# yflyzhang/RankPO

Hardware: AMD Instinct MI355X
Metric: query-passage pairs/sec (higher is better)
Workload: dtype bf16

## Files before the change

rankpo_amd/csrc/encoder_ops.hip:

```cpp
#include "common.hpp"

namespace {

constexpr int kEwThreads = 256;

__device__ __forceinline__ float sigmoid_f(float x) { return 1.0f / (1.0f + __expf(-x)); }

template <typename T>
__global__ __launch_bounds__(kEwThreads) void swiglu_fwd_kernel(const T* __restrict__ g, const T* __restrict__ u,
                                                                T* __restrict__ out, int64_t rows, int vec_per_row,
                                                                int64_t ld_gu, int64_t ld_out) {
    constexpr int V = Elem<T>::kVec;
    const int64_t i = (int64_t)blockIdx.x * kEwThreads + threadIdx.x;
    const int64_t r = i / vec_per_row;
    if (r >= rows) return;
    const int c = (int)(i - r * vec_per_row) * V;
    Vec16<T> a, b, o;
    a.load_nt(g + r * ld_gu + c);
    b.load_nt(u + r * ld_gu + c);
#pragma unroll
    for (int k = 0; k < V; ++k) o.v[k] = a.v[k] * sigmoid_f(a.v[k]) * b.v[k];
    o.store_nt(out + r * ld_out + c);
}

template <typename T>
__global__ __launch_bounds__(kEwThreads) void swiglu_bwd_kernel(const T* g, const T* u, const T* dout, T* dg, T* du,
                                                                T* prod, int64_t rows, int vec_per_row, int64_t ld_gu,
                                                                int64_t ld_dout, int64_t ld_dgu,
                                                                int64_t ld_prod) {
    constexpr int V = Elem<T>::kVec;
    const int64_t i = (int64_t)blockIdx.x * kEwThreads + threadIdx.x;
    const int64_t r = i / vec_per_row;
    if (r >= rows) return;
    const int c = (int)(i - r * vec_per_row) * V;
    Vec16<T> a, b, d, og, ou, op;
    a.load_nt(g + r * ld_gu + c);
    b.load_nt(u + r * ld_gu + c);
    d.load_nt(dout + r * ld_dout + c);
#pragma unroll
    for (int k = 0; k < V; ++k) {
        const float s = sigmoid_f(a.v[k]);
        const float silu = a.v[k] * s;
        og.v[k] = d.v[k] * b.v[k] * (s + silu * (1.0f - s));
        ou.v[k] = d.v[k] * silu;
        op.v[k] = silu * b.v[k];
    }
    og.store_nt(dg + r * ld_dgu + c);
    ou.store_nt(du + r * ld_dgu + c);
    if (prod) op.store_nt(prod + r * ld_prod + c);
}

template <typename T>
__global__ __launch_bounds__(kEwThreads) void rope_kernel(const T* xin, T* x, int64_t row_stride,
                                                          const float* __restrict__ cs, const float* __restrict__ sn,
                                                          int64_t rows, int H, int hd, int64_t period, float sign) {
    constexpr int V = Elem<T>::kVec;
    const int half = hd >> 1;
    const int vec_per_head = half / V;
    const int total = H * vec_per_head;
    const int rpb = total <= kEwThreads / 2 ? kEwThreads / total : 1;
    const int rin = rpb > 1 ? threadIdx.x / total : 0;
    const int i0 = rpb > 1 ? threadIdx.x - rin * total : threadIdx.x;
    if (rin >= rpb) return;
    for (int64_t r = (int64_t)blockIdx.x * rpb + rin; r < rows; r += (int64_t)gridDim.x * rpb) {
        T* xr = x + r * row_stride;
        const T* xi = xin + r * row_stride;
        const float* c = cs + (r % period) * half;
        const float* s = sn + (r % period) * half;
        for (int i = i0; i < total; i += (rpb > 1 ? total : kEwThreads)) {
            const int h = i / vec_per_head, j = (i - h * vec_per_head) * V;
            T* lo = xr + h * hd + j;
            T* hi = lo + half;
            Vec16<T> a, b, oa, ob;
            a.load_nt(xi + h * hd + j);
            b.load_nt(xi + h * hd + j + half);
#pragma unroll
            for (int k = 0; k < V; ++k) {
                const float cc = c[j + k], ss = sign * s[j + k];
                oa.v[k] = a.v[k] * cc - b.v[k] * ss;
                ob.v[k] = b.v[k] * cc + a.v[k] * ss;
            }
            oa.store_nt(lo);
            ob.store_nt(hi);
        }
    }
}

template <typename T, int TC, bool DGU_T>
__global__ __launch_bounds__(256) void swiglu_bwd_t_kernel(const T* __restrict__ g, const T* __restrict__ u, const T* __restrict__ dout,
                                                           T* __restrict__ dg, T* __restrict__ du, T* __restrict__ prod_t,
                                                           T* __restrict__ dgu_t, int64_t rows, int64_t cols, int64_t ld_gu,
                                                           int64_t ld_dout, int64_t ld_dgu, int64_t ld_pt) {
    constexpr int V = Elem<T>::kVec;
    constexpr int TR = 64;
    constexpr int LDT = TC + 8 / (int)sizeof(T);
    constexpr int VPR = TC / V;
    constexpr int VPC = TR / V;
    constexpr int NI = TR * VPR / 256;
    __shared__ __attribute__((aligned(16))) T tile[TR][LDT];
    const int64_t r0 = (int64_t)blockIdx.y * TR, c0 = (int64_t)blockIdx.x * TC;
    const int t = threadIdx.x;
    auto st_tile = [](T* dst, const uint4_t v) {
        uint2_t* d2 = reinterpret_cast<uint2_t*>(dst);
        d2[0] = uint2_t{v.x, v.y};
        d2[1] = uint2_t{v.z, v.w};
    };
    uint4_t pk_g[DGU_T ? NI : 1], pk_u[DGU_T ? NI : 1];
#pragma unroll
    for (int i = 0; i < NI; ++i) {
        const int idx = t + 256 * i;
        const int row = idx / VPR, cv = (idx % VPR) * V;
        const int64_t r = r0 + row, c = c0 + cv;
        __attribute__((aligned(16))) T pv[V];
        __attribute__((aligned(16))) T gv[V];
        __attribute__((aligned(16))) T uv[V];
        if (r < rows && c < cols) {
            Vec16<T> a, b, d, og, ou;
            a.load_nt(g + r * ld_gu + c);
            b.load_nt(u + r * ld_gu + c);
            d.load_nt(dout + r * ld_dout + c);
#pragma unroll
            for (int k = 0; k < V; ++k) {
                const float sg = sigmoid_f(a.v[k]);
                const float silu = a.v[k] * sg;
                og.v[k] = d.v[k] * b.v[k] * (sg + silu * (1.0f - sg));
                ou.v[k] = d.v[k] * silu;
                Elem<T>::st(&pv[k], silu * b.v[k]);
                if constexpr (DGU_T) {
                    Elem<T>::st(&gv[k], og.v[k]);
                    Elem<T>::st(&uv[k], ou.v[k]);
                }
            }
            og.store_nt(dg + r * ld_dgu + c);
            ou.store_nt(du + r * ld_dgu + c);
        } else {
#pragma unroll
            for (int k = 0; k < V; ++k) pv[k] = gv[k] = uv[k] = T(0);
        }
        st_tile(&tile[row][cv], *reinterpret_cast<const uint4_t*>(pv));
        if constexpr (DGU_T) {
            pk_g[i] = *reinterpret_cast<const uint4_t*>(gv);
            pk_u[i] = *reinterpret_cast<const uint4_t*>(uv);
        }
    }
    auto flush = [&](T* __restrict__ out) {
        __syncthreads();
#pragma unroll
        for (int i = 0; i < TC * VPC / 256; ++i) {
            const int idx = t + 256 * i;
            const int oc = idx / VPC, rv = (idx % VPC) * V;
            const int64_t c = c0 + oc, r = r0 + rv;
            if (c >= cols || r >= rows) continue;
            __attribute__((aligned(16))) T v[V];
#pragma unroll
            for (int e = 0; e < V; ++e) v[e] = tile[rv + e][oc];
            if (r + V <= rows) {
                __builtin_nontemporal_store(*reinterpret_cast<const uint4_t*>(v), reinterpret_cast<uint4_t*>(out + c * ld_pt + r));
            } else {
#pragma unroll
                for (int e = 0; e < V; ++e)
                    if (r + e < rows) out[c * ld_pt + r + e] = v[e];
            }
        }
    };
    flush(prod_t);
    if constexpr (DGU_T) {
        auto refill = [&](const uint4_t* pk) {
            __syncthreads();
#pragma unroll
            for (int i = 0; i < NI; ++i) {
                const int idx = t + 256 * i;
                st_tile(&tile[idx / VPR][(idx % VPR) * V], pk[i]);
            }
        };
        refill(pk_g);
        flush(dgu_t);
        refill(pk_u);
        flush(dgu_t + cols * ld_pt);
    }
}

inline unsigned ew_grid(int64_t nvec) { return (unsigned)rpo_cdiv(nvec, kEwThreads); }

}

template <typename T>
__global__ __launch_bounds__(256) void transpose_kernel(const T* __restrict__ in, T* __restrict__ out, int64_t R, int64_t C,
                                                        int64_t ld_in, int64_t ld_out, int vec_in, int vec_out) {
    constexpr int V = 16 / (int)sizeof(T);
    constexpr int TS = 64;
    constexpr int LDT = TS + 8 / (int)sizeof(T);
    constexpr int VPR = TS / V;
    __shared__ __attribute__((aligned(16))) T tile[TS][LDT];
    const int64_t r0 = (int64_t)blockIdx.y * TS, c0 = (int64_t)blockIdx.x * TS;
    const int t = threadIdx.x;
#pragma unroll
    for (int i = 0; i < TS * VPR / 256; ++i) {
        const int idx = t + 256 * i;
        const int row = idx / VPR, cv = (idx % VPR) * V;
        const int64_t r = r0 + row, c = c0 + cv;
        __attribute__((aligned(16))) T v[V];
        if (r < R && vec_in && c + V <= C) {
            *reinterpret_cast<uint4_t*>(v) = __builtin_nontemporal_load(reinterpret_cast<const uint4_t*>(in + r * ld_in + c));
        } else {
#pragma unroll
            for (int e = 0; e < V; ++e) v[e] = (r < R && c + e < C) ? in[r * ld_in + c + e] : T(0);
        }
#pragma unroll
        for (int e = 0; e < V; ++e) tile[row][cv + e] = v[e];
    }
    __syncthreads();
#pragma unroll
    for (int i = 0; i < TS * VPR / 256; ++i) {
        const int idx = t + 256 * i;
        const int oc = idx / VPR, rv = (idx % VPR) * V;
        const int64_t c = c0 + oc, r = r0 + rv;
        if (c >= C) continue;
        __attribute__((aligned(16))) T v[V];
#pragma unroll
        for (int e = 0; e < V; ++e) v[e] = tile[rv + e][oc];
        if (vec_out && r + V <= R) {
            __builtin_nontemporal_store(*reinterpret_cast<const uint4_t*>(v), reinterpret_cast<uint4_t*>(out + c * ld_out + r));
        } else {
#pragma unroll
            for (int e = 0; e < V; ++e)
                if (r + e < R) out[c * ld_out + r + e] = v[e];
        }
    }
}

extern "C" int rpo_transpose(const void* in, void* out, int64_t rows, int64_t cols, int64_t ld_in, int64_t ld_out, int dtype,
                             rpo_stream_t stream) {
    if (!in || !out || rows <= 0 || cols <= 0 || ld_in < cols || ld_out < rows) return RPO_ERR_INVALID_ARG;
    if (!rpo_dtype_ok(dtype)) return RPO_ERR_INVALID_ARG;
    if (dtype == RPO_DT_F16) dtype = RPO_DT_BF16;
    const int64_t gx = rpo_cdiv(cols, 64), gy = rpo_cdiv(rows, 64);
    if (gy > 65535) return RPO_ERR_UNSUPPORTED;
    const int es = dtype == RPO_DT_BF16 ? 2 : 4, V = 16 / es;
    const int vec_in = rpo_aligned16(in) && (ld_in % V == 0), vec_out = rpo_aligned16(out) && (ld_out % V == 0);
    hipStream_t st = (hipStream_t)stream;
    const dim3 grid((unsigned)gx, (unsigned)gy);
    if (dtype == RPO_DT_BF16)
        RPO_LAUNCH(transpose_kernel<bf16_t>, grid, dim3(256), 0, st, (const bf16_t*)in, (bf16_t*)out, rows, cols, ld_in, ld_out,
                   vec_in, vec_out);
    else
        RPO_LAUNCH(transpose_kernel<float>, grid, dim3(256), 0, st, (const float*)in, (float*)out, rows, cols, ld_in, ld_out,
                   vec_in, vec_out);
    return rpo_launch_status();
}

extern "C" int rpo_swiglu_fwd(const void* g, const void* u, void* out, int64_t rows, int64_t cols, int64_t ld_gu,
                              int64_t ld_out, int dtype, rpo_stream_t stream) {
    if (!g || !u || !out || rows <= 0 || cols <= 0) return RPO_ERR_INVALID_ARG;
    const int V = dtype == RPO_DT_BF16 ? 8 : 4;
    if (cols % V != 0 || ld_gu % V != 0 || ld_out % V != 0 || ld_gu < cols || ld_out < cols || !rpo_aligned16(g) ||
        !rpo_aligned16(u) || !rpo_aligned16(out))
        return RPO_ERR_UNSUPPORTED;
    const int64_t nvec = rows * (cols / V);
    if (nvec / kEwThreads >= INT32_MAX) return RPO_ERR_UNSUPPORTED;
    hipStream_t st = (hipStream_t)stream;
    if (dtype == RPO_DT_BF16)
        RPO_LAUNCH(swiglu_fwd_kernel<bf16_t>, dim3(ew_grid(nvec)), dim3(kEwThreads), 0, st, (const bf16_t*)g,
                   (const bf16_t*)u, (bf16_t*)out, rows, (int)(cols / V), ld_gu, ld_out);
    else if (dtype == RPO_DT_F32)
        RPO_LAUNCH(swiglu_fwd_kernel<float>, dim3(ew_grid(nvec)), dim3(kEwThreads), 0, st, (const float*)g,
                   (const float*)u, (float*)out, rows, (int)(cols / V), ld_gu, ld_out);
    else
        return RPO_ERR_INVALID_ARG;
    return rpo_launch_status();
}

extern "C" int rpo_swiglu_bwd(const void* g, const void* u, const void* dout, void* dg, void* du, void* prod_out,
                              int64_t rows, int64_t cols, int64_t ld_gu, int64_t ld_dout, int64_t ld_dgu, int64_t ld_prod,
                              int dtype, rpo_stream_t stream) {
    if (!g || !u || !dout || !dg || !du || rows <= 0 || cols <= 0) return RPO_ERR_INVALID_ARG;
    const int V = dtype == RPO_DT_BF16 ? 8 : 4;
    if (cols % V != 0 || ld_gu % V != 0 || ld_dout % V != 0 || ld_dgu % V != 0 || !rpo_aligned16(g) ||
        !rpo_aligned16(u) || !rpo_aligned16(dout) || !rpo_aligned16(dg) || !rpo_aligned16(du) ||
        (prod_out && (ld_prod % V != 0 || !rpo_aligned16(prod_out))))
        return RPO_ERR_UNSUPPORTED;
    const int64_t nvec = rows * (cols / V);
    if (nvec / kEwThreads >= INT32_MAX) return RPO_ERR_UNSUPPORTED;
    hipStream_t st = (hipStream_t)stream;
    if (dtype == RPO_DT_BF16)
        RPO_LAUNCH(swiglu_bwd_kernel<bf16_t>, dim3(ew_grid(nvec)), dim3(kEwThreads), 0, st, (const bf16_t*)g,
                   (const bf16_t*)u, (const bf16_t*)dout, (bf16_t*)dg, (bf16_t*)du, (bf16_t*)prod_out, rows, (int)(cols / V),
                   ld_gu, ld_dout, ld_dgu, ld_prod);
    else if (dtype == RPO_DT_F32)
        RPO_LAUNCH(swiglu_bwd_kernel<float>, dim3(ew_grid(nvec)), dim3(kEwThreads), 0, st, (const float*)g,
                   (const float*)u, (const float*)dout, (float*)dg, (float*)du, (float*)prod_out, rows, (int)(cols / V), ld_gu,
                   ld_dout, ld_dgu, ld_prod);
    else
        return RPO_ERR_INVALID_ARG;
    return rpo_launch_status();
}

extern "C" int rpo_swiglu_bwd_t(const void* g, const void* u, const void* dout, void* dg, void* du, void* prod_t_out,
                                void* dgu_t_out, int64_t rows, int64_t cols, int64_t ld_gu, int64_t ld_dout, int64_t ld_dgu,
                                int64_t ld_t, int dtype, rpo_stream_t stream) {
    if (!g || !u || !dout || !dg || !du || !prod_t_out || rows <= 0 || cols <= 0) return RPO_ERR_INVALID_ARG;
    const int V = dtype == RPO_DT_BF16 ? 8 : 4;
    if (cols % V != 0 || ld_gu % V != 0 || ld_dout % V != 0 || ld_dgu % V != 0 || ld_t % V != 0 || ld_t < rows ||
        !rpo_aligned16(g) || !rpo_aligned16(u) || !rpo_aligned16(dout) || !rpo_aligned16(dg) || !rpo_aligned16(du) ||
        !rpo_aligned16(prod_t_out) || (dgu_t_out && !rpo_aligned16(dgu_t_out)))
        return RPO_ERR_UNSUPPORTED;
    constexpr int kTC = 256;
    const int64_t gy = rpo_cdiv(rows, 64);
    if (gy > 65535) return RPO_ERR_UNSUPPORTED;
    hipStream_t st = (hipStream_t)stream;
#define RPO_SWT(T, TCV, FLAG)                                                                                               \
    RPO_LAUNCH((swiglu_bwd_t_kernel<T, TCV, FLAG>), dim3((unsigned)rpo_cdiv(cols, TCV), (unsigned)gy), dim3(256), 0, st,    \
               (const T*)g, (const T*)u, (const T*)dout, (T*)dg, (T*)du, (T*)prod_t_out, (T*)dgu_t_out, rows, cols, ld_gu,   \
               ld_dout, ld_dgu, ld_t)
    if (dtype == RPO_DT_BF16) {
        if (dgu_t_out) RPO_SWT(bf16_t, kTC, true);
        else RPO_SWT(bf16_t, kTC, false);
    } else if (dtype == RPO_DT_F32) {
        if (dgu_t_out) RPO_SWT(float, kTC / 2, true);
        else RPO_SWT(float, kTC / 2, false);
    } else {
        return RPO_ERR_INVALID_ARG;
    }
#undef RPO_SWT
    return rpo_launch_status();
}

extern "C" int rpo_rope(const void* x_in, void* x, int64_t row_stride, const float* cos_tab, const float* sin_tab, int64_t rows,
                                int64_t heads, int64_t head_dim, int64_t period, int dtype, int backward,
                                rpo_stream_t stream) {
    if (!x_in || !x || !cos_tab || !sin_tab || rows <= 0 || heads <= 0 || head_dim <= 0 || period <= 0)
        return RPO_ERR_INVALID_ARG;
    const int V = dtype == RPO_DT_BF16 ? 8 : 4;
    if ((head_dim / 2) % V != 0 || head_dim % 2 != 0 || row_stride % V != 0 || !rpo_aligned16(x) || !rpo_aligned16(x_in))
        return RPO_ERR_UNSUPPORTED;
    const int64_t pairs = heads * ((head_dim / 2) / V);
    const int64_t rpb = pairs <= kEwThreads / 2 ? kEwThreads / pairs : 1;
    const int64_t nblk = rpo_cdiv(rows, rpb);
    int64_t grid = nblk < INT32_MAX ? nblk : INT32_MAX;
    hipStream_t st = (hipStream_t)stream;
    const float sign = backward ? -1.0f : 1.0f;
    if (dtype == RPO_DT_BF16)
        RPO_LAUNCH(rope_kernel<bf16_t>, dim3((unsigned)grid), dim3(kEwThreads), 0, st, (const bf16_t*)x_in, (bf16_t*)x, row_stride, cos_tab,
                   sin_tab, rows, (int)heads, (int)head_dim, period, sign);
    else if (dtype == RPO_DT_F32)
        RPO_LAUNCH(rope_kernel<float>, dim3((unsigned)grid), dim3(kEwThreads), 0, st, (const float*)x_in, (float*)x, row_stride, cos_tab,
                   sin_tab, rows, (int)heads, (int)head_dim, period, sign);
    else
        return RPO_ERR_INVALID_ARG;
    return rpo_launch_status();
}

namespace {

constexpr int kNormThreads = 256, kNormWaves = kNormThreads / 64;

template <typename T> struct Raw16 {
    uint4_t r;
    __device__ __forceinline__ void load_nt(const T* p) { r = __builtin_nontemporal_load(reinterpret_cast<const uint4_t*>(p)); }
    __device__ __forceinline__ void load(const T* p) { r = *reinterpret_cast<const uint4_t*>(p); }
    __device__ __forceinline__ float get(int e) const;
};
template <> __device__ __forceinline__ float Raw16<float>::get(int e) const { return __uint_as_float(r[e]); }
template <> __device__ __forceinline__ float Raw16<bf16_t>::get(int e) const {
    return (e & 1) ? __uint_as_float(r[e >> 1] & 0xffff0000u) : __uint_as_float(r[e >> 1] << 16);
}

template <typename T, int KMAX>
__global__ __launch_bounds__(kNormThreads) void add_rmsnorm_fwd_kernel(const T* __restrict__ x, const T* __restrict__ delta,
                                                                       const T* __restrict__ w, float eps,
                                                                       T* __restrict__ x_out, T* __restrict__ y,
                                                                       float* __restrict__ rstd_out, int64_t rows,
                                                                       int d, int64_t rows_per_wave) {
    constexpr int V = Elem<T>::kVec;
    const int lane = threadIdx.x & 63;
    const int64_t wave = (int64_t)blockIdx.x * kNormWaves + (threadIdx.x >> 6);
    const int nvec = d / V;
    float wv[KMAX][V];
#pragma unroll
    for (int k = 0; k < KMAX; ++k) {
        const int vi = lane + 64 * k;
        if (vi < nvec) {
            Vec16<T> t;
            t.load(w + vi * V);
#pragma unroll
            for (int e = 0; e < V; ++e) wv[k][e] = t.v[e];
        }
    }
    const int64_t r0 = wave * rows_per_wave, r1 = r0 + rows_per_wave < rows ? r0 + rows_per_wave : rows;
    const float inv_d = 1.0f / (float)d;
    for (int64_t r = r0; r < r1; ++r) {
        Vec16<T> xv[KMAX];
        float ss = 0.f;
#pragma unroll
        for (int k = 0; k < KMAX; ++k) {
            const int vi = lane + 64 * k;
            if (vi < nvec) {
                xv[k].load_nt(x + r * d + vi * V);
                if (delta) {
                    Vec16<T> dv;
                    dv.load_nt(delta + r * d + vi * V);
#pragma unroll
                    for (int e = 0; e < V; ++e) xv[k].v[e] = Elem<T>::round(xv[k].v[e] + dv.v[e]);
                    xv[k].store(x_out + r * d + vi * V);
                }
#pragma unroll
                for (int e = 0; e < V; ++e) ss = fmaf(xv[k].v[e], xv[k].v[e], ss);
            }
        }
        ss = wave_sum(ss);
        const float rstd = rsqrtf(ss * inv_d + eps);
        if (lane == 0) rstd_out[r] = rstd;
#pragma unroll
        for (int k = 0; k < KMAX; ++k) {
            const int vi = lane + 64 * k;
            if (vi < nvec) {
                Vec16<T> o;
#pragma unroll
                for (int e = 0; e < V; ++e) o.v[e] = xv[k].v[e] * rstd * wv[k][e];
                o.store(y + r * d + vi * V);
            }
        }
    }
}

template <typename T, int KMAX>
__global__ __launch_bounds__(kNormThreads) void add_rmsnorm_bwd_kernel(const T* __restrict__ dy, const T* __restrict__ xn,
                                                                       const T* __restrict__ w,
                                                                       const float* __restrict__ rstd_in,
                                                                       const T* __restrict__ dres, T* __restrict__ dx,
                                                                       float* __restrict__ dw_partial, int64_t rows,
                                                                       int d, int64_t rows_per_wave) {
    constexpr int V = Elem<T>::kVec;
    const int lane = threadIdx.x & 63;
    const int64_t wave = (int64_t)blockIdx.x * kNormWaves + (threadIdx.x >> 6);
    const int nvec = d / V;
    float dwa[KMAX][V];
    Raw16<T> wv[KMAX];
#pragma unroll
    for (int k = 0; k < KMAX; ++k) {
        const int vi = lane + 64 * k;
#pragma unroll
        for (int e = 0; e < V; ++e) dwa[k][e] = 0.f;
        if (vi < nvec) wv[k].load(w + vi * V);
    }
    const int64_t r0 = wave * rows_per_wave, r1 = r0 + rows_per_wave < rows ? r0 + rows_per_wave : rows;
    const float inv_d = 1.0f / (float)d;
    for (int64_t r = r0; r < r1; ++r) {
        const float rstd = rstd_in[r];
        Raw16<T> gv[KMAX], xv[KMAX], rv[KMAX];
        float c = 0.f;
#pragma unroll
        for (int k = 0; k < KMAX; ++k) {
            const int vi = lane + 64 * k;
            if (vi < nvec) {
                gv[k].load_nt(dy + r * d + vi * V);
                xv[k].load_nt(xn + r * d + vi * V);
                if (dres) rv[k].load_nt(dres + r * d + vi * V);
            }
        }
#pragma unroll
        for (int k = 0; k < KMAX; ++k) {
            const int vi = lane + 64 * k;
            if (vi < nvec) {
#pragma unroll
                for (int e = 0; e < V; ++e) {
                    const float xh = xv[k].get(e) * rstd;
                    const float dyv = gv[k].get(e);
                    dwa[k][e] = fmaf(dyv, xh, dwa[k][e]);
                    c = fmaf(dyv * wv[k].get(e), xh, c);
                }
            }
        }
        c = wave_sum(c) * inv_d;
#pragma unroll
        for (int k = 0; k < KMAX; ++k) asm volatile("" : "+v"(gv[k].r), "+v"(xv[k].r), "+v"(wv[k].r));
#pragma unroll
        for (int k = 0; k < KMAX; ++k) {
            const int vi = lane + 64 * k;
            if (vi < nvec) {
                Vec16<T> o;
#pragma unroll
                for (int e = 0; e < V; ++e) {
                    const float xh = xv[k].get(e) * rstd;
                    const float g = gv[k].get(e) * wv[k].get(e);
                    o.v[e] = (g - xh * c) * rstd;
                }
                if (dres) {
#pragma unroll
                    for (int e = 0; e < V; ++e) o.v[e] += rv[k].get(e);
                }
                o.store(dx + r * d + vi * V);
            }
        }
    }
    if (r0 < rows || true) {
#pragma unroll
        for (int k = 0; k < KMAX; ++k) {
            const int vi = lane + 64 * k;
            if (vi < nvec) {
                Vec16<float> o;
#pragma unroll
                for (int h = 0; h < V / 4; ++h) {
#pragma unroll
                    for (int e = 0; e < 4; ++e) o.v[e] = dwa[k][4 * h + e];
                    o.store(dw_partial + wave * d + vi * V + 4 * h);
                }
            }
        }
    }
}

template <typename T>
int launch_norm_fwd(const void* x, const void* delta, const void* w, float eps, void* x_out, void* y, float* rstd,
                    int64_t rows, int64_t d, int nwaves, hipStream_t st) {
    constexpr int V = Elem<T>::kVec;
    const int kk = (int)rpo_cdiv(d / V, 64);
    const int64_t rpw = rpo_cdiv(rows, nwaves);
    const dim3 grid((unsigned)rpo_cdiv(nwaves, kNormWaves)), block(kNormThreads);
#define RPO_NF(K)                                                                                               \
    RPO_LAUNCH((add_rmsnorm_fwd_kernel<T, K>), grid, block, 0, st, (const T*)x, (const T*)delta, (const T*)w, eps, \
               (T*)x_out, (T*)y, rstd, rows, (int)d, rpw)
    if (kk <= 1) RPO_NF(1);
    else if (kk <= 2) RPO_NF(2);
    else if (kk <= 4) RPO_NF(4);
    else if (kk <= 8) RPO_NF(8);
    else if (kk <= 16) RPO_NF(16);
    else return RPO_ERR_UNSUPPORTED;
#undef RPO_NF
    return rpo_launch_status();
}

template <typename T>
int launch_norm_bwd(const void* dy, const void* xn, const void* w, const float* rstd, const void* dres, void* dx,
                    float* dwp, int64_t rows, int64_t d, int nwaves, hipStream_t st) {
    constexpr int V = Elem<T>::kVec;
    const int kk = (int)rpo_cdiv(d / V, 64);
    const int64_t rpw = rpo_cdiv(rows, nwaves);
    const dim3 grid((unsigned)rpo_cdiv(nwaves, kNormWaves)), block(kNormThreads);
#define RPO_NB(K)                                                                                                \
    RPO_LAUNCH((add_rmsnorm_bwd_kernel<T, K>), grid, block, 0, st, (const T*)dy, (const T*)xn, (const T*)w, rstd,  \
               (const T*)dres, (T*)dx, dwp, rows, (int)d, rpw)
    if (kk <= 1) RPO_NB(1);
    else if (kk <= 2) RPO_NB(2);
    else if (kk <= 4) RPO_NB(4);
    else if (kk <= 8) RPO_NB(8);
    else return RPO_ERR_UNSUPPORTED;
#undef RPO_NB
    return rpo_launch_status();
}

}

#ifndef RPO_NORM_FWD_CAP
#define RPO_NORM_FWD_CAP 8192
#endif
#ifndef RPO_NORM_BWD_CAP
#define RPO_NORM_BWD_CAP 8192
#endif
static int norm_waves(int64_t rows, int64_t cap) {
    int64_t w = rows < cap ? rows : cap;
    w = (w + 3) / 4 * 4;
    return (int)(w < 4 ? 4 : w);
}

extern "C" int rpo_add_rmsnorm_waves(int64_t rows) {
    return norm_waves(rows, RPO_NORM_BWD_CAP);
}

extern "C" int rpo_add_rmsnorm_fwd(const void* x, const void* delta, const void* weight, float eps, void* x_out,
                                   void* y_out, float* rstd_out, int64_t rows, int64_t d, int dtype,
                                   rpo_stream_t stream) {
    if (!x || !weight || !y_out || !rstd_out || rows <= 0 || d <= 0) return RPO_ERR_INVALID_ARG;
    if (delta && !x_out) return RPO_ERR_INVALID_ARG;
    const int V = dtype == RPO_DT_BF16 ? 8 : 4;
    if (d % V != 0 || !rpo_aligned16(x) || !rpo_aligned16(y_out) || !rpo_aligned16(weight) ||
        (delta && (!rpo_aligned16(delta) || !rpo_aligned16(x_out))))
        return RPO_ERR_UNSUPPORTED;
    hipStream_t st = (hipStream_t)stream;
    const int nw = norm_waves(rows, RPO_NORM_FWD_CAP);
    if (dtype == RPO_DT_BF16) return launch_norm_fwd<bf16_t>(x, delta, weight, eps, x_out, y_out, rstd_out, rows, d, nw, st);
    if (dtype == RPO_DT_F32) return launch_norm_fwd<float>(x, delta, weight, eps, x_out, y_out, rstd_out, rows, d, nw, st);
    return RPO_ERR_INVALID_ARG;
}

extern "C" int rpo_add_rmsnorm_bwd(const void* dy, const void* x_new, const void* weight, const float* rstd,
                                   const void* dres, void* dx_out, float* dw_partial, int64_t rows, int64_t d,
                                   int dtype, rpo_stream_t stream) {
    if (!dy || !x_new || !weight || !rstd || !dx_out || !dw_partial || rows <= 0 || d <= 0) return RPO_ERR_INVALID_ARG;
    const int V = dtype == RPO_DT_BF16 ? 8 : 4;
    if (d % V != 0 || !rpo_aligned16(dy) || !rpo_aligned16(x_new) || !rpo_aligned16(dx_out) || !rpo_aligned16(weight) ||
        !rpo_aligned16(dw_partial) || (dres && !rpo_aligned16(dres)))
        return RPO_ERR_UNSUPPORTED;
    hipStream_t st = (hipStream_t)stream;
    const int nw = rpo_add_rmsnorm_waves(rows);
    if (dtype == RPO_DT_BF16) return launch_norm_bwd<bf16_t>(dy, x_new, weight, rstd, dres, dx_out, dw_partial, rows, d, nw, st);
    if (dtype == RPO_DT_F32) return launch_norm_bwd<float>(dy, x_new, weight, rstd, dres, dx_out, dw_partial, rows, d, nw, st);
    return RPO_ERR_INVALID_ARG;
}
```

Before: 55.34.

## Add wide-tile transpose kernel and prefetching interleaved rmsnorm forward

Adds a transpose kernel with a 64xwide tile, used when the grid is large enough, so each block moves more data and needs fewer launches. The add-rmsnorm forward kernel now interleaves rows across waves with a grid stride and prefetches the next row's inputs in raw form while the current row is reduced, to hide load latency. The forward wave cap rises to allow more waves. This raises register and LDS use and makes the access pattern more complex.

Measured after the change: 55.38 (median of 6 runs). No clear change (+0.1%).

```diff
diff --git a/rankpo_amd/csrc/encoder_ops.hip b/rankpo_amd/csrc/encoder_ops.hip
--- a/rankpo_amd/csrc/encoder_ops.hip
+++ b/rankpo_amd/csrc/encoder_ops.hip
@@ -229,6 +229,58 @@
     }
 }
 
+template <typename T>
+__global__ __launch_bounds__(256) void transpose_wide_kernel(const T* __restrict__ in, T* __restrict__ out, int64_t R, int64_t C,
+                                                             int64_t ld_in, int64_t ld_out, int vec_in, int vec_out) {
+    constexpr int V = 16 / (int)sizeof(T);
+    constexpr int TR = 64, TC = 512 / (int)sizeof(T);
+    constexpr int LDT = TC + 8 / (int)sizeof(T);
+    constexpr int VPR = TC / V;
+    constexpr int VPC = TR / V;
+    __shared__ __attribute__((aligned(16))) T tile[TR][LDT];
+    const int64_t r0 = (int64_t)blockIdx.y * TR, c0 = (int64_t)blockIdx.x * TC;
+    const int t = threadIdx.x;
+#pragma unroll
+    for (int i = 0; i < TR * VPR / 256; ++i) {
+        const int idx = t + 256 * i;
+        const int row = idx / VPR, cv = (idx % VPR) * V;
+        const int64_t r = r0 + row, c = c0 + cv;
+        __attribute__((aligned(16))) T v[V];
+        if (r < R && vec_in && c + V <= C) {
+            *reinterpret_cast<uint4_t*>(v) = __builtin_nontemporal_load(reinterpret_cast<const uint4_t*>(in + r * ld_in + c));
+        } else {
+#pragma unroll
+            for (int e = 0; e < V; ++e) v[e] = (r < R && c + e < C) ? in[r * ld_in + c + e] : T(0);
+        }
+        const uint4_t pk = *reinterpret_cast<const uint4_t*>(v);
+        uint2_t* d2 = reinterpret_cast<uint2_t*>(&tile[row][cv]);
+        d2[0] = uint2_t{pk.x, pk.y};
+        d2[1] = uint2_t{pk.z, pk.w};
+    }
+    __syncthreads();
+#pragma unroll
+    for (int i = 0; i < TC * VPC / 256; ++i) {
+        const int idx = t + 256 * i;
+        const int oc = idx / VPC, rv = (idx % VPC) * V;
+        const int64_t c = c0 + oc, r = r0 + rv;
+        if (c >= C || r >= R) continue;
+        __attribute__((aligned(16))) T v[V];
+#pragma unroll
+        for (int e = 0; e < V; ++e) v[e] = tile[rv + e][oc];
+        if (vec_out && r + V <= R) {
+            __builtin_nontemporal_store(*reinterpret_cast<const uint4_t*>(v), reinterpret_cast<uint4_t*>(out + c * ld_out + r));
+        } else {
+#pragma unroll
+            for (int e = 0; e < V; ++e)
+                if (r + e < R) out[c * ld_out + r + e] = v[e];
+        }
+    }
+}
+
+#ifndef RPO_TRANSPOSE_WIDE_MIN_BLOCKS
+#define RPO_TRANSPOSE_WIDE_MIN_BLOCKS 1024
+#endif
+
 extern "C" int rpo_transpose(const void* in, void* out, int64_t rows, int64_t cols, int64_t ld_in, int64_t ld_out, int dtype,
                              rpo_stream_t stream) {
     if (!in || !out || rows <= 0 || cols <= 0 || ld_in < cols || ld_out < rows) return RPO_ERR_INVALID_ARG;
@@ -239,6 +291,17 @@
     const int es = dtype == RPO_DT_BF16 ? 2 : 4, V = 16 / es;
     const int vec_in = rpo_aligned16(in) && (ld_in % V == 0), vec_out = rpo_aligned16(out) && (ld_out % V == 0);
     hipStream_t st = (hipStream_t)stream;
+    const int64_t wgx = rpo_cdiv(cols, 512 / es);
+    if (wgx * gy >= (int64_t)RPO_TRANSPOSE_WIDE_MIN_BLOCKS && cols > 64) {
+        const dim3 wgrid((unsigned)wgx, (unsigned)gy);
+        if (dtype == RPO_DT_BF16)
+            RPO_LAUNCH(transpose_wide_kernel<bf16_t>, wgrid, dim3(256), 0, st, (const bf16_t*)in, (bf16_t*)out, rows, cols, ld_in,
+                       ld_out, vec_in, vec_out);
+        else
+            RPO_LAUNCH(transpose_wide_kernel<float>, wgrid, dim3(256), 0, st, (const float*)in, (float*)out, rows, cols, ld_in,
+                       ld_out, vec_in, vec_out);
+        return rpo_launch_status();
+    }
     const dim3 grid((unsigned)gx, (unsigned)gy);
     if (dtype == RPO_DT_BF16)
         RPO_LAUNCH(transpose_kernel<bf16_t>, grid, dim3(256), 0, st, (const bf16_t*)in, (bf16_t*)out, rows, cols, ld_in, ld_out,
@@ -365,6 +428,14 @@
     return (e & 1) ? __uint_as_float(r[e >> 1] & 0xffff0000u) : __uint_as_float(r[e >> 1] << 16);
 }
 
+#ifndef RPO_NORM_FWD_ILV
+#define RPO_NORM_FWD_ILV 1
+#endif
+#ifndef RPO_NORM_FWD_MODE
+#define RPO_NORM_FWD_MODE 1
+#endif
+template <int KMAX> constexpr int norm_mode(int mode) { return KMAX <= 4 ? mode : 0; }
+
 template <typename T, int KMAX>
 __global__ __launch_bounds__(kNormThreads) void add_rmsnorm_fwd_kernel(const T* __restrict__ x, const T* __restrict__ delta,
                                                                        const T* __restrict__ w, float eps,
@@ -386,27 +457,13 @@
             for (int e = 0; e < V; ++e) wv[k][e] = t.v[e];
         }
     }
-    const int64_t r0 = wave * rows_per_wave, r1 = r0 + rows_per_wave < rows ? r0 + rows_per_wave : rows;
+    constexpr int MODE = norm_mode<KMAX>(RPO_NORM_FWD_MODE);
+    constexpr bool ILV = RPO_NORM_FWD_ILV;
+    const int64_t rs = ILV ? (int64_t)gridDim.x * kNormWaves : 1;
+    const int64_t r0 = ILV ? wave : wave * rows_per_wave;
+    const int64_t r1 = ILV ? rows : (r0 + rows_per_wave < rows ? r0 + rows_per_wave : rows);
     const float inv_d = 1.0f / (float)d;
-    for (int64_t r = r0; r < r1; ++r) {
-        Vec16<T> xv[KMAX];
-        float ss = 0.f;
-#pragma unroll
-        for (int k = 0; k < KMAX; ++k) {
-            const int vi = lane + 64 * k;
-            if (vi < nvec) {
-                xv[k].load_nt(x + r * d + vi * V);
-                if (delta) {
-                    Vec16<T> dv;
-                    dv.load_nt(delta + r * d + vi * V);
-#pragma unroll
-                    for (int e = 0; e < V; ++e) xv[k].v[e] = Elem<T>::round(xv[k].v[e] + dv.v[e]);
-                    xv[k].store(x_out + r * d + vi * V);
-                }
-#pragma unroll
-                for (int e = 0; e < V; ++e) ss = fmaf(xv[k].v[e], xv[k].v[e], ss);
-            }
-        }
+    auto finish = [&](int64_t r, const Vec16<T>* xv, float ss) {
         ss = wave_sum(ss);
         const float rstd = rsqrtf(ss * inv_d + eps);
         if (lane == 0) rstd_out[r] = rstd;
@@ -419,6 +476,63 @@
                 for (int e = 0; e < V; ++e) o.v[e] = xv[k].v[e] * rstd * wv[k][e];
                 o.store(y + r * d + vi * V);
             }
+        }
+    };
+    if constexpr (MODE == 1) {
+        Raw16<T> px[KMAX], pd[KMAX];
+        auto fetch = [&](int64_t r) {
+#pragma unroll
+            for (int k = 0; k < KMAX; ++k) {
+                const int vi = lane + 64 * k;
+                if (vi < nvec) {
+                    px[k].load_nt(x + r * d + vi * V);
+                    if (delta) pd[k].load_nt(delta + r * d + vi * V);
+                }
+            }
+        };
+        if (r0 < r1) fetch(r0);
+        for (int64_t r = r0; r < r1; r += rs) {
+            Vec16<T> xv[KMAX];
+            float ss = 0.f;
+#pragma unroll
+            for (int k = 0; k < KMAX; ++k) {
+                const int vi = lane + 64 * k;
+                if (vi < nvec) {
+#pragma unroll
+                    for (int e = 0; e < V; ++e) xv[k].v[e] = px[k].get(e);
+                    if (delta) {
+#pragma unroll
+                        for (int e = 0; e < V; ++e) xv[k].v[e] = Elem<T>::round(xv[k].v[e] + pd[k].get(e));
+                        xv[k].store(x_out + r * d + vi * V);
+                    }
+#pragma unroll
+                    for (int e = 0; e < V; ++e) ss = fmaf(xv[k].v[e], xv[k].v[e], ss);
+                }
+            }
+            if (r + rs < r1) fetch(r + rs);
+            finish(r, xv, ss);
+        }
+    } else {
+        for (int64_t r = r0; r < r1; r += rs) {
+            Vec16<T> xv[KMAX];
+            float ss = 0.f;
+#pragma unroll
+            for (int k = 0; k < KMAX; ++k) {
+                const int vi = lane + 64 * k;
+                if (vi < nvec) {
+                    xv[k].load_nt(x + r * d + vi * V);
+                    if (delta) {
+                        Vec16<T> dv;
+                        dv.load_nt(delta + r * d + vi * V);
+#pragma unroll
+                        for (int e = 0; e < V; ++e) xv[k].v[e] = Elem<T>::round(xv[k].v[e] + dv.v[e]);
+                        xv[k].store(x_out + r * d + vi * V);
+                    }
+#pragma unroll
+                    for (int e = 0; e < V; ++e) ss = fmaf(xv[k].v[e], xv[k].v[e], ss);
+                }
+            }
+            finish(r, xv, ss);
         }
     }
 }
@@ -552,7 +666,7 @@
 }
 
 #ifndef RPO_NORM_FWD_CAP
-#define RPO_NORM_FWD_CAP 8192
+#define RPO_NORM_FWD_CAP 32768
 #endif
 #ifndef RPO_NORM_BWD_CAP
 #define RPO_NORM_BWD_CAP 8192
```
